# WU-CVGL/Styl3R

Measured on AMD Instinct MI355X. Metric: 256x256 stylized views/sec (fwd+bwd) @ ~65k Gaussians, higher is better.
Workload: dtype f32; 1 GPU; rasterizer fwd+bwd (decoder API + MSE, the loss computed inside the composite kernels): 10 scenes x 4 target views/GPU/step, 256x256, G=65536 Gaussians/scene (1 ctx view x 256x256), sh_degree=0, make_scale_invariant, all views in one batched launch; outputs the decoder discards are not computed (decoder_splatting_cuda.py:37-68 drops radii / opacity / n_touched, MSE sends no depth gradient: the com; parallelism=dp1 (scenes sharded)

## Files before the change

### include/gsr.h

```cpp
#ifndef GSR_H
#define GSR_H

#include <stddef.h>
#include <stdint.h>

#ifdef __cplusplus
extern "C" {
#endif

#define GSR_OK 0
#define GSR_EINVAL (-1)
#define GSR_ENOSPACE (-2)
#define GSR_ELAUNCH (-3)

#define GSR_TILE 16
#define GSR_VIEW_FLOATS 64

typedef struct GsrView {
    float viewmatrix[16];
    float projmatrix[16];
    float projmatrix_raw[16];
    float campos[3];
    float tanfovx, tanfovy;
    float bg[3];
    float scale;
    float pad[7];
} GsrView;

typedef struct GsrDims {
    int32_t B;
    int32_t Vt;
    int32_t G;
    int32_t H, W;
    int32_t M;
    int32_t sh_degree;
    int32_t flags;
    void *profile;
} GsrDims;

#define GSR_FLAG_NTOUCHED 1
#define GSR_FLAG_COV9 2
#define GSR_FLAG_PHASE_BIN 4
#define GSR_FLAG_PHASE_RENDER 8

#define GSR_FLAG_PREZERO_GRADS 16
#define GSR_FLAG_BIN_BALLOT 32
#define GSR_FLAG_SORT_KEYS_SHIFT 8

#define GSR_STATUS_WORDS 8
#define GSR_ST_PAIRS 0
#define GSR_ST_OVERFLOW 1
#define GSR_ST_MAX_TILE 2
#define GSR_ST_PAIRS_HI 3

typedef struct GsrLayout {
    size_t records;
    size_t tile_count;
    size_t tile_offset;
    size_t tile_cursor;
    size_t pairs;
    size_t point_list;
    size_t final_T;
    size_t n_contrib;
    size_t grad_rec;
    size_t status;
    size_t tile_order;
    size_t pairs_alt;
    size_t loss_partial;
    size_t loss_ticket;
    size_t loss_diff;
    size_t total;
} GsrLayout;

#define GSR_ID_MASK 0x0fffffffu
#define GSR_QUAD_SHIFT 28

int gsr_workspace_layout(const GsrDims *dims, int64_t pair_capacity, GsrLayout *out);

int gsr_forward(const GsrDims *dims, const GsrView *views, const float *means, const float *cov6,
                const float *opac, const float *shs, int64_t pair_capacity, void *workspace,
                size_t workspace_bytes, float *image, float *depth, float *opacity, int32_t *radii,
                int32_t *n_touched, int32_t *status, void *stream);

int gsr_backward(const GsrDims *dims, const GsrView *views, const float *means, const float *cov6,
                 const float *shs, int64_t pair_capacity, void *workspace, size_t workspace_bytes,
                 const float *dL_dimage, const float *dL_ddepth, float *dL_dmeans, float *dL_dcov6,
                 float *dL_dopac, float *dL_dshs, float *dL_dmeans2D, float *dL_dtau, void *stream);

typedef struct GsrFused {
    uint32_t *tile_count;
    const float *mse_target;
    float mse_weight;
    float *mse_loss;
    const float *mse_grad_loss;
} GsrFused;
int gsr_forward_fused(const GsrDims *dims, const GsrView *views, const float *means, const float *cov6,
                      const float *opac, const float *shs, int64_t pair_capacity, void *workspace,
                      size_t workspace_bytes, float *image, float *depth, float *opacity, int32_t *radii,
                      int32_t *n_touched, int32_t *status, const GsrFused *fx, void *stream);
int gsr_backward_fused(const GsrDims *dims, const GsrView *views, const float *means, const float *cov6,
                       const float *shs, int64_t pair_capacity, void *workspace, size_t workspace_bytes,
                       const float *dL_dimage, const float *dL_ddepth, float *dL_dmeans, float *dL_dcov6,
                       float *dL_dopac, float *dL_dshs, float *dL_dmeans2D, float *dL_dtau, const GsrFused *fx,
// ... 34 lines not shown
```

### styl3r_amd/_lib.py

```python
from __future__ import annotations

import ctypes as C
import os
import subprocess
from pathlib import Path

_PKG = Path(__file__).resolve().parent
_CSRC = _PKG / "csrc"
_LIBDIR = _PKG / "lib"
LIB_PATH = _LIBDIR / os.environ.get("GSR_LIB_NAME", "libgsr_hip.so")

_SOURCES = ["gsr_forward.hip", "gsr_backward.hip", "gsr_api.hip", "gsr_loss.hip"]
_HEADERS = ["gsr_common.h", "../../include/gsr.h"]

HIPCC_FLAGS = [
    "--offload-arch=gfx950", "-O3", "-std=c++17", "-fPIC", "-shared",
    "-fhip-fp32-correctly-rounded-divide-sqrt", "-fvisibility=hidden",
    "-fno-slp-vectorize",
]


def _hipcc() -> str:
    for cand in (os.environ.get("HIPCC"), "/opt/rocm/bin/hipcc"):
        if cand and os.path.exists(cand):
# ... 18 lines not shown


def build_digest() -> str:
    _, deps, cmd = _build_cmd()
    return sources_digest(deps, cmd)


def built_digest() -> str:
    stamp = LIB_PATH.with_suffix(".stamp")
    return stamp.read_text().strip() if stamp.exists() and LIB_PATH.exists() else ""


def build_library(force: bool = False, verbose: bool = False) -> Path:
    srcs, deps, cmd = _build_cmd()
    _LIBDIR.mkdir(exist_ok=True)
    want = sources_digest(deps, cmd)
    if not force and built_digest() == want:
        return LIB_PATH
    real = [_hipcc(), *cmd[1:-2], "-o", str(LIB_PATH)]
    if verbose:
        print(" ".join(real))
    subprocess.run(real, check=True, cwd=str(_CSRC))
    LIB_PATH.with_suffix(".stamp").write_text(want)
    return LIB_PATH


class GsrDims(C.Structure):
    _fields_ = [("B", C.c_int32), ("Vt", C.c_int32), ("G", C.c_int32), ("H", C.c_int32), ("W", C.c_int32),
                ("M", C.c_int32), ("sh_degree", C.c_int32), ("flags", C.c_int32), ("profile", C.c_void_p)]


class GsrLayout(C.Structure):
    _fields_ = [(n, C.c_size_t) for n in ("records", "tile_count", "tile_offset", "tile_cursor", "pairs", "point_list",
                                          "final_T", "n_contrib", "grad_rec", "status", "tile_order", "pairs_alt", "loss_partial", "loss_ticket", "loss_diff", "total")]


class GsrFused(C.Structure):
    _fields_ = [("tile_count", C.c_void_p), ("mse_target", C.c_void_p), ("mse_weight", C.c_float), ("mse_loss", C.c_void_p),
                ("mse_grad_loss", C.c_void_p)]


GSR_FLAG_NTOUCHED = 1
GSR_FLAG_COV9 = 2
GSR_FLAG_PHASE_BIN = 4
GSR_FLAG_PHASE_RENDER = 8
GSR_FLAG_PREZERO_GRADS = 16
GSR_FLAG_BIN_BALLOT = 32
GSR_ID_MASK = 0x0FFFFFFF
GSR_QUAD_SHIFT = 28
GSR_FLAG_SORT_KEYS_SHIFT = 8
GSR_STATUS_WORDS = 8
GSR_VIEW_FLOATS = 64
GSR_N_STAGES = 7
STAGE_NAMES = ("preprocess", "scan_tiles", "scatter", "tile_sort", "composite_fwd", "composite_bwd", "preprocess_bwd")
EXPORTS = ("gsr_workspace_layout", "gsr_forward", "gsr_backward", "gsr_forward_fused", "gsr_backward_fused", "gsr_version", "gsr_profile_create",
           "gsr_profile_destroy", "gsr_profile_read", "gsr_profile_set_stages", "gsr_last_error", "gsr_build_views", "gsr_mse_scratch_bytes",
           "gsr_mse_forward", "gsr_mse_backward")
ERRORS = {-1: "GSR_EINVAL (bad dimension / null pointer / unsupported degree)",
          -2: "GSR_ENOSPACE (workspace too small)", -3: "GSR_ELAUNCH (kernel launch failed)"}

_lib = None


def load() -> C.CDLL:
    global _lib
    if _lib is not None:
        return _lib
    if not LIB_PATH.exists():
        raise RuntimeError(
            f"{LIB_PATH} is missing: the HIP rasterizer has not been built. "
            "Run `python -c 'import __graft_entry__ as g; g.build()'` (needs hipcc). There is no CPU fallback.")
    import torch
    lib = C.CDLL(str(LIB_PATH))
    vp, i64, sz = C.c_void_p, C.c_int64, C.c_size_t
    lib.gsr_workspace_layout.argtypes = [C.POINTER(GsrDims), i64, C.POINTER(GsrLayout)]
    lib.gsr_workspace_layout.restype = C.c_int
    lib.gsr_forward.argtypes = [C.POINTER(GsrDims), vp, vp, vp, vp, vp, i64, vp, sz, vp, vp, vp, vp, vp, vp, vp]
    lib.gsr_forward.restype = C.c_int
    lib.gsr_backward.argtypes = [C.POINTER(GsrDims), vp, vp, vp, vp, i64, vp, sz, vp, vp, vp, vp, vp, vp, vp, vp, vp]
    lib.gsr_backward.restype = C.c_int
    lib.gsr_forward_fused.argtypes = [C.POINTER(GsrDims), vp, vp, vp, vp, vp, i64, vp, sz, vp, vp, vp, vp, vp, vp, C.POINTER(GsrFused), vp]
    lib.gsr_forward_fused.restype = C.c_int
    lib.gsr_backward_fused.argtypes = [C.POINTER(GsrDims), vp, vp, vp, vp, i64, vp, sz, vp, vp, vp, vp, vp, vp, vp, vp, C.POINTER(GsrFused), vp]
    lib.gsr_backward_fused.restype = C.c_int
# ... 56 lines not shown
```

### styl3r_amd/csrc/gsr_api.hip

```cpp
#include <new>

#include "gsr_common.h"

namespace gsr {
int layout(const GsrDims &d, long long cap, GsrLayout &L);
int forward(const GsrDims &d, const GsrView *views, const float *means, const float *cov6, const float *opac,
            const float *shs, long long cap, void *workspace, size_t workspace_bytes, float *image, float *depth,
            float *opacity, int32_t *radii, int32_t *n_touched, int32_t *status, const GsrFused *fx, hipStream_t stream);
int backward(const GsrDims &d, const GsrView *views, const float *means, const float *cov6, const float *shs,
             long long cap, void *workspace, size_t workspace_bytes, const float *dL_dimage, const float *dL_ddepth,
             float *dL_dmeans, float *dL_dcov6, float *dL_dopac, float *dL_dshs, float *dL_dmeans2D, float *dL_dtau,
             const GsrFused *fx, hipStream_t stream);
}

namespace gsr {
thread_local hipError_t g_last_hip_error = hipSuccess;

#pragma clang fp contract(off)
__device__ inline void inverse4(const float *m, float *inv)
{
    float a[4][8];
#pragma unroll
    for (int r = 0; r < 4; ++r)
#pragma unroll
// ... 195 lines not shown
    if (!p) return;
    const size_t n = (size_t)p->max_calls * GSR_N_STAGES * 2;
    for (size_t i = 0; i < n; ++i)
        if (p->ev[i]) (void)hipEventDestroy(p->ev[i]);
    delete[] p->ev;
    delete p;
}

__attribute__((visibility("default"))) int gsr_profile_read(GsrProfile *p, float *ms_sum, int32_t *count)
{
    if (!p || !ms_sum || !count) return GSR_EINVAL;
    for (int s = 0; s < GSR_N_STAGES; ++s) { ms_sum[s] = 0.f; count[s] = 0; }
    for (int s = 0; s < GSR_N_STAGES; ++s) {
        if (!((p->mask >> s) & 1u)) continue;
        const int n = (s <= GSR_STAGE_COMPOSITE_FWD) ? p->next_fwd : p->next_bwd;
        for (int c = 0; c < n; ++c) {
            float ms = 0.f;
            if (hipEventSynchronize(p->at(c, s, 1)) != hipSuccess) return GSR_ELAUNCH;
            if (hipEventElapsedTime(&ms, p->at(c, s, 0), p->at(c, s, 1)) != hipSuccess) return GSR_ELAUNCH;
            ms_sum[s] += ms; count[s] += 1;
        }
    }
    p->next_fwd = p->next_bwd = 0;
    return GSR_OK;
}

__attribute__((visibility("default"))) int gsr_profile_set_stages(GsrProfile *p, uint32_t stage_mask)
{
    if (!p || p->next_fwd || p->next_bwd) return GSR_EINVAL;
    p->mask = stage_mask & ((1u << GSR_N_STAGES) - 1u);
    return GSR_OK;
}

__attribute__((visibility("default"))) const char *gsr_version(void) { return "gsr-hip gfx950 0.6.0"; }

}
```

### styl3r_amd/csrc/gsr_backward.hip

```cpp
#include <type_traits>

#include "gsr_common.h"

namespace gsr {

enum { GR_RGB = 0, GR_DEPTH = 3, GR_MX = 4, GR_MY = 5, GR_CA = 6, GR_CB = 7, GR_CC = 8, GR_OP = 9 };

template <bool DEPTH>
__global__ void __launch_bounds__(64) k_composite_bwd(GsrDims d, const GsrView *__restrict__ views, Ptrs ws,
                                                     const float *__restrict__ dL_dimage,
                                                     const float *__restrict__ dL_ddepth,
                                                     bool mse, float mse_weight, const float *__restrict__ mse_grad_loss)
{
    if (ws.status[GSR_ST_OVERFLOW]) return;
    __shared__ float4 s_q[64 * 3];

    const int gx = tiles_x(d.W), T = gx * tiles_y(d.H);
    const uint32_t tv = ws.tile_order[blockIdx.y * gridDim.x + blockIdx.x];
    const int tile = (int)(tv % (uint32_t)T), v = (int)(tv / (uint32_t)T);
    const int lane = threadIdx.x;
    const int ox = (tile % gx) * TILE + (lane & 7), oy = (tile / gx) * TILE + (lane >> 3);
    const size_t P = (size_t)d.H * d.W;

    const size_t t = (size_t)v * T + tile;
    const uint32_t start = ws.tile_offset[t], end = ws.tile_offset[t + 1];
    if (start == end) return;
    const uint32_t *__restrict__ plist = ws.point_list + start;
    const SplatRec *__restrict__ recs = ws.records + (size_t)v * d.G;
    float *grad = ws.grad_rec + (size_t)v * d.G * GR_STRIDE;
    const GsrView &vw = views[v];

    const float fx0 = (float)ox, fy0 = (float)oy;
    float Tr[4], g0[4], g1[4], g2[4], gd[4], S[4];
    uint32_t last[4];
    uint32_t mx = 0;
    const float mse_c = mse ? 2.0f * mse_weight / (float)((size_t)d.B * d.Vt * 3 * P) * (mse_grad_loss ? mse_grad_loss[0] : 1.f) : 0.f;
#pragma unroll
    for (int k = 0; k < 4; ++k) {
        const int px = ox + (k & 1) * 8, py = oy + (k >> 1) * 8;
        const bool inside = px < d.W && py < d.H;
        const size_t pix = (size_t)py * d.W + px;
        const float Tf = inside ? ws.final_T[v * P + pix] : 0.f;
        last[k] = inside ? ws.n_contrib[v * P + pix] : 0u;
        g0[k] = (inside && dL_dimage) ? dL_dimage[(v * 3 + 0) * P + pix] : 0.f;
        g1[k] = (inside && dL_dimage) ? dL_dimage[(v * 3 + 1) * P + pix] : 0.f;
        g2[k] = (inside && dL_dimage) ? dL_dimage[(v * 3 + 2) * P + pix] : 0.f;
        if (mse && inside) {
            const float e0 = mse_c * ws.loss_diff[(v * 3 + 0) * P + pix], e1 = mse_c * ws.loss_diff[(v * 3 + 1) * P + pix],
                        e2 = mse_c * ws.loss_diff[(v * 3 + 2) * P + pix];
            if (dL_dimage) { g0[k] += e0; g1[k] += e1; g2[k] += e2; }
            else { g0[k] = e0; g1[k] = e1; g2[k] = e2; }
        }
        gd[k] = (DEPTH && inside) ? dL_ddepth[v * P + pix] : 0.f;
        S[k] = Tf * (vw.bg[0] * g0[k] + vw.bg[1] * g1[k] + vw.bg[2] * g2[k]);
        Tr[k] = Tf;
        mx = max(mx, last[k]);
    }
    const float ddelx_dx = 0.5f * (float)d.W, ddely_dy = 0.5f * (float)d.H;
#pragma unroll
    for (int o = 32; o > 0; o >>= 1) mx = max(mx, (uint32_t)__shfl_xor((int)mx, o, 64));
    const int max_last = __builtin_amdgcn_readfirstlane((int)mx);
    constexpr bool NINE = !DEPTH;
    int slot;
    if (NINE) { const int i9 = reduce9_slot(lane); slot = i9 < 0 ? -1 : (i9 < 3 ? i9 : i9 + 1); }
    else slot = reduce10_slot(lane);

    for (int hi = max_last; hi > 0; hi -= 64) {
        const int cnt = min(64, hi);
        asm volatile("" ::: "memory");
        uint32_t bm = 0;
        if (lane < cnt) {
            const uint32_t word = plist[hi - 1 - lane];
            bm = word >> GSR_QUAD_SHIFT;
            stage_entry_bwd(recs, word & GSR_ID_MASK, bm, s_q + lane * 3);
        }
        unsigned long long todo = __builtin_amdgcn_ballot_w64(bm != 0u);
        asm volatile("s_waitcnt lgkmcnt(0)" ::: "memory");
        for (; todo; todo &= todo - 1ull) {
            const int j = __builtin_ctzll(todo);
            const uint32_t entry = (uint32_t)(hi - 1 - j);
            const float4 a = s_q[j * 3 + 0];
            const float4 b = s_q[j * 3 + 1];
            const float4 c = s_q[j * 3 + 2];
            const uint32_t quad = __builtin_amdgcn_readfirstlane(__float_as_uint(c.w));
            float s[10];
#pragma unroll
            for (int i = 0; i < 10; ++i) asm volatile("" : "=v"(s[i]));
            if (!DEPTH && !NINE) s[GR_DEPTH] = 0.f;
            unsigned long long anym = 0ull;
            auto eval = [&](const bool FIRST, const int k) {
                const float dx = (a.x - fx0) - (float)((k & 1) * 8), dy = (a.y - fy0) - (float)((k >> 1) * 8);
                const float power = -0.5f * (a.z * dx * dx + b.x * dy * dy) - a.w * dx * dy;
                const float Graw = footprint_exp(power);
                const float araw = fminf(0.99f, b.y * Graw);
                const unsigned long long vm = __builtin_amdgcn_ballot_w64(entry < last[k]) & __builtin_amdgcn_ballot_w64(power <= 0.f) &
                                              __builtin_amdgcn_ballot_w64(araw >= (1.f / 255.f));
                anym |= vm;
                const float alpha = sel0_f(vm, araw);
                const float Gv = sel0_f(vm, Graw);
                const float inv = __builtin_amdgcn_rcpf(1.f - alpha);
                Tr[k] *= inv;
// ... 277 lines not shown
        for (int k = 0; k < 3 * NC; ++k) dsh[k] = dsh_acc[k];
        for (int k = 3 * NC; k < ncol; ++k) dsh[k] = 0.f;
    }
}
#pragma clang fp contract(fast)

int layout(const GsrDims &d, long long cap, GsrLayout &L);
Ptrs carve(void *base, const GsrLayout &L);

int backward(const GsrDims &d, const GsrView *views, const float *means, const float *cov6, const float *shs,
             long long cap, void *workspace, size_t workspace_bytes, const float *dL_dimage, const float *dL_ddepth,
             float *dL_dmeans, float *dL_dcov6, float *dL_dopac, float *dL_dshs, float *dL_dmeans2D, float *dL_dtau,
             const GsrFused *fx, hipStream_t stream)
{
    GsrLayout L;
    int rc = layout(d, cap, L);
    if (rc != GSR_OK) return rc;
    const float *mse_target = fx ? fx->mse_target : nullptr;
    if (!views || !means || !cov6 || !shs || !workspace || !dL_dmeans || !dL_dcov6 || !dL_dopac || !dL_dshs) return GSR_EINVAL;
    if (!dL_dimage && !mse_target) return GSR_EINVAL;
    if (workspace_bytes < L.total) return GSR_ENOSPACE;
    Ptrs ws = carve(workspace, L);
    const int V = d.B * d.Vt, T = tiles_x(d.W) * tiles_y(d.H);
    (void)hipGetLastError();
    StageTimer tm(d.profile, false, stream);
    if (!(d.flags & GSR_FLAG_PREZERO_GRADS) &&
        !hip_ok(hipMemsetAsync(ws.grad_rec, 0, (size_t)V * d.G * GR_STRIDE * 4, stream))) return GSR_ELAUNCH;
    if (dL_dtau && !hip_ok(hipMemsetAsync(dL_dtau, 0, (size_t)V * 6 * 4, stream))) return GSR_ELAUNCH;
    tm.begin(GSR_STAGE_COMPOSITE_BWD);
    {
        const float *mg = fx ? fx->mse_grad_loss : nullptr;
        const float mw = fx ? fx->mse_weight : 0.f;
        const bool mse = mse_target != nullptr;
        if (dL_ddepth) hipLaunchKernelGGL(k_composite_bwd<true>, dim3(T, V), dim3(64), 0, stream, d, views, ws, dL_dimage, dL_ddepth, mse, mw, mg);
        else hipLaunchKernelGGL(k_composite_bwd<false>, dim3(T, V), dim3(64), 0, stream, d, views, ws, dL_dimage, dL_ddepth, mse, mw, mg);
    }
    tm.end(GSR_STAGE_COMPOSITE_BWD); tm.begin(GSR_STAGE_PREPROCESS_BWD);
    const dim3 gG((d.G + 255) / 256, d.B);
#define GSR_LAUNCH_K7(DEG) hipLaunchKernelGGL(k_preprocess_bwd<DEG>, gG, dim3(256), 0, stream, d, views, means, cov6, shs, ws, \
                                              dL_dmeans, dL_dcov6, dL_dopac, dL_dshs, dL_dmeans2D, dL_dtau)
    switch (d.M > 0 ? d.sh_degree : -1) {
        case -1: GSR_LAUNCH_K7(-1); break;
        case 0: GSR_LAUNCH_K7(0); break;
        case 1: GSR_LAUNCH_K7(1); break;
        case 2: GSR_LAUNCH_K7(2); break;
        case 3: GSR_LAUNCH_K7(3); break;
        default: GSR_LAUNCH_K7(4); break;
    }
#undef GSR_LAUNCH_K7
    tm.end(GSR_STAGE_PREPROCESS_BWD);
    return launch_status();
}

}
```

### styl3r_amd/csrc/gsr_common.h

```cpp
#pragma once
#include <hip/hip_runtime.h>
#include <stdint.h>

#include "../../include/gsr.h"

namespace gsr {

constexpr int TILE = GSR_TILE;
constexpr int TILE_PIX = TILE * TILE;
constexpr int WAVE = 64;

struct alignas(16) SplatRec {
    float x, y, depth;
    uint32_t rad_flags;
    float A, B, C, opacity;
    float r, g, b;
    uint32_t ext;
};
constexpr int LDS_TILES_MAX = 4096;
static_assert(sizeof(SplatRec) == 48, "SplatRec must be 48 bytes");

struct alignas(16) QueueRec {
    float x, y, A, B;
    float C, opacity, depth; uint32_t id;
    float r, g, b; uint32_t quad;
};
static_assert(sizeof(QueueRec) == 48, "QueueRec must be 48 bytes");

constexpr int GR_STRIDE = 12;

struct Ptrs {
    SplatRec *records;
    uint32_t *tile_count, *tile_offset, *tile_cursor, *tile_order;
    unsigned long long *pairs, *pairs_alt;
    uint32_t *point_list;
    float *loss_partial;
    uint32_t *loss_ticket;
    float *loss_diff;
    float *final_T;
    uint32_t *n_contrib;
    float *grad_rec;
    int32_t *status;
};

}

struct GsrProfile {
    int max_calls;
    int next_fwd, next_bwd;
    uint32_t mask;
    hipEvent_t *ev;
    hipEvent_t &at(int call, int stage, int which) { return ev[((size_t)call * GSR_N_STAGES + stage) * 2 + which]; }
};

namespace gsr {

extern thread_local hipError_t g_last_hip_error;
inline int launch_status()
{
    hipError_t e = hipGetLastError();
    if (e == hipSuccess) return GSR_OK;
    g_last_hip_error = e;
    return GSR_ELAUNCH;
}
inline bool hip_ok(hipError_t e)
{
    if (e == hipSuccess) return true;
    g_last_hip_error = e;
    return false;
}

struct StageTimer {
    GsrProfile *p; int slot; hipStream_t s;
    StageTimer(void *prof, bool fwd, hipStream_t stream, bool resume = false)
        : p(static_cast<GsrProfile *>(prof)), slot(-1), s(stream)
    {
        if (!p) return;
        int &n = fwd ? p->next_fwd : p->next_bwd;
        if (resume) { if (n > 0 && n <= p->max_calls) slot = n - 1; }
        else if (n < p->max_calls) slot = n++;
    }
    void begin(int stage) { if (slot >= 0 && ((p->mask >> stage) & 1u)) (void)hipEventRecord(p->at(slot, stage, 0), s); }
    void end(int stage) { if (slot >= 0 && ((p->mask >> stage) & 1u)) (void)hipEventRecord(p->at(slot, stage, 1), s); }
};

__host__ __device__ inline int tiles_x(int W) { return (W + TILE - 1) / TILE; }
__host__ __device__ inline int tiles_y(int H) { return (H + TILE - 1) / TILE; }

__device__ constexpr float SH_C0 = 0.28209479177387814f;
__device__ constexpr float SH_C1 = 0.4886025119029199f;
__device__ constexpr float SH_C2_0 = 1.0925484305920792f, SH_C2_1 = -1.0925484305920792f, SH_C2_2 = 0.31539156525252005f,
                           SH_C2_3 = -1.0925484305920792f, SH_C2_4 = 0.5462742152960396f;
__device__ constexpr float SH_C3_0 = -0.5900435899266435f, SH_C3_1 = 2.890611442640554f, SH_C3_2 = -0.4570457994644658f,
                           SH_C3_3 = 0.3731763325901154f, SH_C3_4 = -0.4570457994644658f, SH_C3_5 = 1.445305721320277f,
                           SH_C3_6 = -0.5900435899266435f;
__device__ constexpr float SH_C4_0 = 2.5033429417967046f, SH_C4_1 = -1.7701307697799304f, SH_C4_2 = 0.9461746957575601f,
                           SH_C4_3 = -0.6690465435572892f, SH_C4_4 = 0.10578554691520431f, SH_C4_5 = -0.6690465435572892f,
                           SH_C4_6 = 0.47308734787878004f, SH_C4_7 = -1.7701307697799304f, SH_C4_8 = 0.6258357354491761f;

#pragma clang fp contract(off)

__device__ inline void sh_basis(int deg, float x, float y, float z, float *b)
{
    b[0] = SH_C0;
    if (deg < 1) return;
    b[1] = -SH_C1 * y; b[2] = SH_C1 * z; b[3] = -SH_C1 * x;
    if (deg < 2) return;
    float xx = x * x, yy = y * y, zz = z * z, xy = x * y, yz = y * z, xz = x * z;
    b[4] = SH_C2_0 * xy; b[5] = SH_C2_1 * yz; b[6] = SH_C2_2 * (2.0f * zz - xx - yy);
    b[7] = SH_C2_3 * xz; b[8] = SH_C2_4 * (xx - yy);
    if (deg < 3) return;
    b[9] = SH_C3_0 * y * (3.0f * xx - yy);
    b[10] = SH_C3_1 * xy * z;
    b[11] = SH_C3_2 * y * (4.0f * zz - xx - yy);
    b[12] = SH_C3_3 * z * (2.0f * zz - 3.0f * xx - 3.0f * yy);
    b[13] = SH_C3_4 * x * (4.0f * zz - xx - yy);
    b[14] = SH_C3_5 * z * (xx - yy);
    b[15] = SH_C3_6 * x * (xx - 3.0f * yy);
    if (deg < 4) return;
    b[16] = SH_C4_0 * xy * (xx - yy);
// ... 305 lines not shown
```

### styl3r_amd/csrc/gsr_forward.hip

```cpp
#include <cstdlib>
#include <cstring>
#include <type_traits>

#include "gsr_common.h"

namespace gsr {

#pragma clang fp contract(off)
template <int DEG>
__global__ void __launch_bounds__(256) k_preprocess(GsrDims d, const GsrView *__restrict__ views,
                                                    const float *__restrict__ means, const float *__restrict__ cov6,
                                                    const float *__restrict__ opac, const float *__restrict__ shs,
                                                    Ptrs ws, int32_t *__restrict__ radii, int lds_tiles)
{
    extern __shared__ uint32_t s_tiles[];
    const int g = blockIdx.x * blockDim.x + threadIdx.x;
    const int b = blockIdx.y;
    const bool live = g < d.G;
    const size_t sg = (size_t)b * d.G + (live ? g : 0);
    const float m0[3] = {means[3 * sg], means[3 * sg + 1], means[3 * sg + 2]};
    float S0[6];
    load_cov(cov6, sg, (d.flags & GSR_FLAG_COV9) != 0, S0);
    const float op = opac[sg];
    const int gx = tiles_x(d.W), gy = tiles_y(d.H), T = gx * gy;
// ... 78 lines not shown
            const int rw = maxx - minx, area = ok ? rw * (maxy - miny) : 0;
            for (int k = 0; k < area; ++k) atomicAdd(&s_tiles[(miny + k / rw) * gx + minx + k % rw], 1u);
            __syncthreads();
            uint32_t *cnt = ws.tile_count + (size_t)v * T;
            for (int t = threadIdx.x; t < T; t += 256) {
                const uint32_t c = s_tiles[t];
                if (c) { atomicAdd(cnt + t, c); s_tiles[t] = 0u; }
            }
            __syncthreads();
        } else {
            const int rw = maxx - minx, area = ok ? rw * (maxy - miny) : 0;
            int amax = area;
#pragma unroll
            for (int o = 32; o > 0; o >>= 1) amax = max(amax, __shfl_xor(amax, o, 64));
            uint32_t *cnt = ws.tile_count + (size_t)v * T;
            for (int k = 0; k < amax; ++k) {
                const bool has = k < area;
                const int ty = has ? miny + k / rw : 0, tx = has ? minx + k % rw : 0;
                wave_agg_inc<false>(cnt, (uint32_t)(ty * gx + tx), has);
            }
        }
        if (live) {
            float4 *dst = reinterpret_cast<float4 *>(ws.records + vg);
            const float4 *src = reinterpret_cast<const float4 *>(&rec);
            dst[0] = src[0]; dst[1] = src[1]; dst[2] = src[2];
            radii[vg] = rad * (ok ? 1 : 0);
        }
    }
}
#pragma clang fp contract(fast)

constexpr int SCAN_PER_MAX = 16;

__global__ void __launch_bounds__(1024) k_scan_tiles(int n, long long capacity, Ptrs ws, int32_t *__restrict__ status, int rearm, int nticket)
{
    __shared__ unsigned long long s_wave[16];
    __shared__ unsigned long long s_carry;
    __shared__ uint32_t s_max[16];
    __shared__ uint32_t s_bin[256], s_shift;
    __shared__ uint32_t s_cnt[1024 * SCAN_PER_MAX];
    const int tid = threadIdx.x, lane = tid & 63, wid = tid >> 6;
    uint32_t mx = 0;
    const int per = (n + 1023) / 1024;
    const bool fast = per <= SCAN_PER_MAX;
    uint32_t c[SCAN_PER_MAX];
    if (fast) {
        for (int i = tid; i < per * 1024; i += 1024) s_cnt[i] = (i < n) ? ws.tile_count[i] : 0u;
        if (rearm) for (int i = tid; i < n; i += 1024) ws.tile_count[i] = 0u;
        for (int i = tid; i < nticket; i += 1024) ws.loss_ticket[i] = 0u;
        __syncthreads();
        unsigned long long tot = 0;
#pragma unroll
        for (int e = 0; e < SCAN_PER_MAX; ++e) {
            c[e] = (e < per) ? s_cnt[tid * per + e] : 0u;
            mx = max(mx, c[e]);
            tot += c[e];
        }
        unsigned long long x = tot;
#pragma unroll
        for (int o = 1; o < 64; o <<= 1) {
            unsigned long long y = __shfl_up(x, o, 64);
            if (lane >= o) x += y;
        }
        if (lane == 63) s_wave[wid] = x;
        __syncthreads();
        unsigned long long off = x - tot;
        for (int w = 0; w < wid; ++w) off += s_wave[w];
        if (tid == 1023) s_carry = off + tot;
#pragma unroll
        for (int e = 0; e < SCAN_PER_MAX; ++e) {
            const int i = tid * per + e;
            if (e < per && i < n) {
// ... 4 lines not shown
        }
    } else {
        if (tid == 0) s_carry = 0;
        for (int i = tid; i < nticket; i += 1024) ws.loss_ticket[i] = 0u;
        __syncthreads();
        for (int base = 0; base < n; base += 1024) {
            int i = base + tid;
            uint32_t cc = (i < n) ? ws.tile_count[i] : 0u;
            mx = max(mx, cc);
            unsigned long long x = cc;
#pragma unroll
            for (int o = 1; o < 64; o <<= 1) {
                unsigned long long y = __shfl_up(x, o, 64);
                if (lane >= o) x += y;
            }
            if (lane == 63) s_wave[wid] = x;
            __syncthreads();
            unsigned long long wave_off = 0;
            for (int w = 0; w < wid; ++w) wave_off += s_wave[w];
            unsigned long long carry = s_carry;
            unsigned long long excl = carry + wave_off + x - cc;
            if (i < n) {
                ws.tile_offset[i] = (uint32_t)min(excl, (unsigned long long)0xffffffffu);
                ws.tile_cursor[i] = 0u;
            }
            __syncthreads();
            if (tid == 1023) s_carry = carry + wave_off + x;
            __syncthreads();
        }
    }
#pragma unroll
    for (int o = 32; o > 0; o >>= 1) mx = max(mx, (uint32_t)__shfl_xor((int)mx, o, 64));
    if (lane == 0) s_max[wid] = mx;
    if (tid < 256) s_bin[tid] = 0u;
    __syncthreads();
    if (tid == 0) {
        uint32_t m = 0;
        for (int w = 0; w < 16; ++w) m = max(m, s_max[w]);
        unsigned long long R = s_carry;
        ws.tile_offset[n] = (uint32_t)min(R, (unsigned long long)0xffffffffu);
        int ovf = (R > (unsigned long long)capacity || R > 0xffffffffull) ? 1 : 0;
        int32_t st[GSR_STATUS_WORDS] = {(int32_t)(R & 0xffffffffull), ovf, (int32_t)m, (int32_t)(R >> 32), 0, 0, 0, 0};
        for (int k = 0; k < GSR_STATUS_WORDS; ++k) { status[k] = st[k]; ws.status[k] = st[k]; }
        uint32_t sh = 0;
        while ((m >> sh) > 255u) ++sh;
        s_shift = sh;
    }
    __syncthreads();
    const uint32_t sh = s_shift;
    if (fast) {
#pragma unroll
        for (int e = 0; e < SCAN_PER_MAX; ++e)
            if (e < per && tid * per + e < n) atomicAdd(&s_bin[255u - min(c[e] >> sh, 255u)], 1u);
    } else {
        for (int i = tid; i < n; i += 1024) atomicAdd(&s_bin[255u - min(ws.tile_count[i] >> sh, 255u)], 1u);
    }
    __syncthreads();
    if (tid < 64) {
        uint32_t b0 = s_bin[tid * 4], b1 = s_bin[tid * 4 + 1], b2 = s_bin[tid * 4 + 2], b3 = s_bin[tid * 4 + 3];
        uint32_t t4 = b0 + b1 + b2 + b3, x = t4;
#pragma unroll
        for (int o = 1; o < 64; o <<= 1) {
            uint32_t y = (uint32_t)__shfl_up((int)x, o, 64);
            if (lane >= o) x += y;
        }
        uint32_t off = x - t4;
        s_bin[tid * 4] = off; s_bin[tid * 4 + 1] = off + b0; s_bin[tid * 4 + 2] = off + b0 + b1; s_bin[tid * 4 + 3] = off + b0 + b1 + b2;
    }
    __syncthreads();
    if (fast) {
#pragma unroll
        for (int e = 0; e < SCAN_PER_MAX; ++e) {
            const int i = tid * per + e;
            if (e < per && i < n) ws.tile_order[atomicAdd(&s_bin[255u - min(c[e] >> sh, 255u)], 1u)] = (uint32_t)i;
        }
    } else {
        for (int i = tid; i < n; i += 1024) {
            const uint32_t pos = atomicAdd(&s_bin[255u - min(ws.tile_count[i] >> sh, 255u)], 1u);
            ws.tile_order[pos] = (uint32_t)i;
            if (rearm) ws.tile_count[i] = 0u;
        }
    }
}

#pragma clang fp contract(off)
__global__ void __launch_bounds__(256) k_scatter(GsrDims d, Ptrs ws)
{
    if (ws.status[GSR_ST_OVERFLOW]) return;
    const int g = blockIdx.x * blockDim.x + threadIdx.x;
    const int v = blockIdx.y;
    const bool live = g < d.G;
    const size_t vg = (size_t)v * d.G + (live ? g : 0);
    const float4 q0 = reinterpret_cast<const float4 *>(ws.records + vg)[0];
    const int rad = live ? (int)(__float_as_uint(q0.w) & 0xffffffu) : 0;
    const int gx = tiles_x(d.W), gy = tiles_y(d.H), T = gx * gy;
    int minx = 0, miny = 0, maxx = 0, maxy = 0;
    if (rad > 0) tile_rect(q0.x, q0.y, rad, gx, gy, minx, miny, maxx, maxy);
    const unsigned long long key = ((unsigned long long)__float_as_uint(q0.z) << 32) | (unsigned)g;
    const size_t tb = (size_t)v * T;
    const int rw = maxx - minx, area = rw * (maxy - miny);
    int amax = area;
#pragma unroll
    for (int o = 32; o > 0; o >>= 1) amax = max(amax, __shfl_xor(amax, o, 64));
    for (int k = 0; k < amax; ++k) {
        const bool has = k < area;
        const int ty = has ? miny + k / rw : 0, tx = has ? minx + k % rw : 0;
        const uint32_t tl = (uint32_t)(ty * gx + tx);
        const uint32_t slot = wave_agg_inc<true>(ws.tile_cursor + tb, tl, has);
        if (has) ws.pairs[ws.tile_offset[tb + tl] + slot] = key;
    }
}
#pragma clang fp contract(fast)
// ... 280 lines not shown
    const int tile = (int)(tv % (uint32_t)T), v = (int)(tv / (uint32_t)T);
    const int lane = threadIdx.x;
    const int ox = (tile % gx) * TILE + (lane & 7), oy = (tile / gx) * TILE + (lane >> 3);

    if (d.flags & GSR_FLAG_PREZERO_GRADS) {
        const size_t n4 = (size_t)d.B * d.Vt * d.G * (GR_STRIDE / 4);
        const size_t nwg = (size_t)gridDim.x * gridDim.y, wg = (size_t)blockIdx.y * gridDim.x + blockIdx.x;
        const size_t per = (n4 + nwg - 1) / nwg, lo = wg * per, hi = lo + per < n4 ? lo + per : n4;
        float4 *gz = reinterpret_cast<float4 *>(ws.grad_rec);
        for (size_t i = lo + lane; i < hi; i += 64) gz[i] = make_float4(0.f, 0.f, 0.f, 0.f);
    }

    const size_t t = (size_t)v * T + tile;
    const uint32_t start = ws.tile_offset[t];
    const int n = (int)(ws.tile_offset[t + 1] - start);
    uint32_t *__restrict__ plist = ws.point_list + start;
    const SplatRec *__restrict__ recs = ws.records + (size_t)v * d.G;
    const int tile_ox = (tile % gx) * TILE, tile_oy = (tile / gx) * TILE;

    float fx0 = (float)ox, fy0 = (float)oy;
    asm volatile("" : "+v"(fx0), "+v"(fy0));
    float Tr[4], C0[4], C1[4], C2[4], D[4], O[4];
    uint32_t last[4];
    bool inside[4];
    unsigned long long dmask[4];
#pragma unroll
    for (int k = 0; k < 4; ++k) {
        const int px = ox + (k & 1) * 8, py = oy + (k >> 1) * 8;
        inside[k] = px < d.W && py < d.H;
        Tr[k] = 1.f; C0[k] = C1[k] = C2[k] = D[k] = O[k] = 0.f;
        last[k] = 0;
        dmask[k] = __builtin_amdgcn_ballot_w64(!inside[k]);
    }

    for (int base = 0; base < n; base += 64) {
        const int cnt = __builtin_amdgcn_readfirstlane(min(64, n - base));
        __syncthreads();
        uint32_t qm = 0;
        if (lane < cnt) {
            const uint32_t id = plist[base + lane] & GSR_ID_MASK;
            qm = stage_entry_fwd(recs, id, tile_ox, tile_oy, s_q + lane * 3);
            if (qm) plist[base + lane] = id | (qm << GSR_QUAD_SHIFT);
        }
        __syncthreads();

        for (unsigned long long todo = __builtin_amdgcn_ballot_w64(qm != 0u); todo; todo &= todo - 1ull) {
            const int j = __builtin_ctzll(todo);
            const float4 a = s_q[j * 3 + 0];
            const float4 b = s_q[j * 3 + 1];
            const float4 c = s_q[j * 3 + 2];
            const uint32_t quad = __builtin_amdgcn_readfirstlane(__float_as_uint(c.w));
            uint32_t touched_tot = 0;
#pragma unroll
            for (int k = 0; k < 4; ++k) {
                if (!(quad & (1u << k))) continue;
                if (dmask[k] == ~0ull) continue;
                const float dx = (a.x - fx0) - (float)((k & 1) * 8), dy = (a.y - fy0) - (float)((k >> 1) * 8);
                const float power = -0.5f * (a.z * dx * dx + b.x * dy * dy) - a.w * dx * dy;
                const float alpha = fminf(0.99f, b.y * footprint_exp(power));
                const float test_T = Tr[k] * (1.f - alpha);
                const unsigned long long live = __builtin_amdgcn_ballot_w64(!(power > 0.f)) & __builtin_amdgcn_ballot_w64(!(alpha < (1.f / 255.f))) & ~dmask[k];
                const unsigned long long keep = __builtin_amdgcn_ballot_w64(!(test_T < 0.0001f));
                dmask[k] |= live & ~keep;
                const unsigned long long comp = live & keep;
                const float w = sel0_f(comp, alpha * Tr[k]);
                C0[k] += c.x * w; C1[k] += c.y * w; C2[k] += c.z * w;
                D[k] += b.z * w;
                O[k] += w;
                if (NTOUCH) touched_tot += (uint32_t)__popcll(comp & __builtin_amdgcn_ballot_w64(test_T > 0.5f));
                Tr[k] = sel_f(comp, test_T, Tr[k]);
                last[k] = sel_u(comp, (uint32_t)(base + j + 1), last[k]);
            }
            if (NTOUCH) {
                if (touched_tot && lane == 0) atomicAdd(n_touched + (size_t)v * d.G + (__float_as_uint(b.w)), (int)touched_tot);
            }
        }
        if ((dmask[0] & dmask[1] & dmask[2] & dmask[3]) == ~0ull) break;
    }

    const size_t P = (size_t)d.H * d.W;
    const GsrView &vw = views[v];
    float sq = 0.f;
#pragma unroll
    for (int k = 0; k < 4; ++k) {
        if (!inside[k]) continue;
        const size_t pix = (size_t)(oy + (k >> 1) * 8) * d.W + (ox + (k & 1) * 8);
        ws.final_T[v * P + pix] = Tr[k];
        ws.n_contrib[v * P + pix] = last[k];
        const float r0 = C0[k] + Tr[k] * vw.bg[0], r1 = C1[k] + Tr[k] * vw.bg[1], r2 = C2[k] + Tr[k] * vw.bg[2];
        image[(v * 3 + 0) * P + pix] = r0;
        image[(v * 3 + 1) * P + pix] = r1;
        image[(v * 3 + 2) * P + pix] = r2;
        out_depth[v * P + pix] = D[k];
        out_opacity[v * P + pix] = O[k];
        if (mse_target) {
            const float e0 = r0 - mse_target[(v * 3 + 0) * P + pix], e1 = r1 - mse_target[(v * 3 + 1) * P + pix],
                        e2 = r2 - mse_target[(v * 3 + 2) * P + pix];
            sq += (e0 * e0 + e1 * e1) + e2 * e2;
            ws.loss_diff[(v * 3 + 0) * P + pix] = e0; ws.loss_diff[(v * 3 + 1) * P + pix] = e1; ws.loss_diff[(v * 3 + 2) * P + pix] = e2;
        }
    }
    if (!mse_target) return;
    const int V = d.B * d.Vt;
    sq = wave_sum_to_lane63(sq);
    uint32_t arrived = 0;
    if (lane == 63) {
        agent_publish(ws.loss_partial + t, sq);
        asm volatile("s_waitcnt vmcnt(0)" ::: "memory");
        arrived = __hip_atomic_fetch_add(ws.loss_ticket + v, 1u, __ATOMIC_RELAXED, __HIP_MEMORY_SCOPE_AGENT);
    }
    arrived = (uint32_t)__builtin_amdgcn_readlane((int)arrived, 63);
    if (arrived != (uint32_t)T - 1u) return;
    float s1 = 0.f;
    for (int i = lane; i < T; i += 64) s1 += agent_read(ws.loss_partial + (size_t)v * T + i);
    s1 = wave_sum_to_lane63(s1);
    arrived = 0;
    if (lane == 63) {
        agent_publish(ws.loss_partial + (size_t)V * T + v, s1);
        asm volatile("s_waitcnt vmcnt(0)" ::: "memory");
        arrived = __hip_atomic_fetch_add(ws.loss_ticket + V, 1u, __ATOMIC_RELAXED, __HIP_MEMORY_SCOPE_AGENT);
    }
    arrived = (uint32_t)__builtin_amdgcn_readlane((int)arrived, 63);
    if (arrived != (uint32_t)V - 1u) return;
    float s2 = 0.f;
    for (int i = lane; i < V; i += 64) s2 += agent_read(ws.loss_partial + (size_t)V * T + i);
    s2 = wave_sum_to_lane63(s2);
    if (lane == 63) mse_loss[0] = mse_weight * (s2 / (float)((size_t)V * 3 * P));
}

static inline size_t align_up(size_t x, size_t a) { return (x + a - 1) / a * a; }

int layout(const GsrDims &d, long long cap, GsrLayout &L)
{
    if (d.B <= 0 || d.Vt <= 0 || d.G <= 0 || d.H <= 0 || d.W <= 0 || cap <= 0) return GSR_EINVAL;
    if (d.M < 0 || d.sh_degree < 0 || d.sh_degree > 4) return GSR_EINVAL;
    if (d.M > 0 && (d.sh_degree + 1) * (d.sh_degree + 1) > d.M) return GSR_EINVAL;
    if (d.M == 0 && d.sh_degree != 0) return GSR_EINVAL;
    if (cap > 0xffffffffll) return GSR_EINVAL;
    if ((long long)d.G * (long long)sizeof(SplatRec) > 0xffffffffll) return GSR_EINVAL;
    static_assert((0xffffffffull / sizeof(SplatRec)) < GSR_ID_MASK, "ids must leave the quadrant-mask bits of a point_list word free");
    const size_t V = (size_t)d.B * d.Vt, T = (size_t)tiles_x(d.W) * tiles_y(d.H), P = (size_t)d.H * d.W;
    size_t off = 0;
    auto take = [&](size_t bytes) { size_t o = off; off = align_up(off + bytes, 256); return o; };
    L.records = take(V * d.G * sizeof(SplatRec));
    L.tile_count = take(V * T * 4);
    L.tile_offset = take((V * T + 1) * 4);
    L.tile_cursor = take(V * T * 4);
    L.pairs = take((size_t)cap * 8);
    L.point_list = take((size_t)cap * 4);
    L.final_T = take(V * P * 4);
    L.n_contrib = take(V * P * 4);
    L.grad_rec = take(V * d.G * 12 * 4);
    L.status = take(GSR_STATUS_WORDS * 4);
    L.tile_order = take(V * T * 4);
    L.pairs_alt = take((size_t)cap * 8);
    L.loss_partial = take((V * T + V) * 4);
    L.loss_ticket = take((V + 1) * 4);
    L.loss_diff = take(V * 3 * P * 4);
    L.total = off;
    return GSR_OK;
}

Ptrs carve(void *base, const GsrLayout &L)
{
    char *p = static_cast<char *>(base);
    Ptrs w;
    w.records = reinterpret_cast<SplatRec *>(p + L.records);
    w.tile_count = reinterpret_cast<uint32_t *>(p + L.tile_count);
    w.tile_offset = reinterpret_cast<uint32_t *>(p + L.tile_offset);
    w.tile_cursor = reinterpret_cast<uint32_t *>(p + L.tile_cursor);
    w.pairs = reinterpret_cast<unsigned long long *>(p + L.pairs);
    w.point_list = reinterpret_cast<uint32_t *>(p + L.point_list);
    w.final_T = reinterpret_cast<float *>(p + L.final_T);
    w.n_contrib = reinterpret_cast<uint32_t *>(p + L.n_contrib);
    w.grad_rec = reinterpret_cast<float *>(p + L.grad_rec);
    w.status = reinterpret_cast<int32_t *>(p + L.status);
    w.tile_order = reinterpret_cast<uint32_t *>(p + L.tile_order);
    w.pairs_alt = reinterpret_cast<unsigned long long *>(p + L.pairs_alt);
    w.loss_partial = reinterpret_cast<float *>(p + L.loss_partial);
    w.loss_ticket = reinterpret_cast<uint32_t *>(p + L.loss_ticket);
    w.loss_diff = reinterpret_cast<float *>(p + L.loss_diff);
    return w;
}

int forward(const GsrDims &d, const GsrView *views, const float *means, const float *cov6, const float *opac,
            const float *shs, long long cap, void *workspace, size_t workspace_bytes, float *image, float *depth,
            float *opacity, int32_t *radii, int32_t *n_touched, int32_t *status, const GsrFused *fx, hipStream_t stream)
{
    GsrLayout L;
    int rc = layout(d, cap, L);
    if (rc != GSR_OK) return rc;
    if (!views || !means || !cov6 || !opac || !shs || !workspace || !image || !depth || !opacity || !radii || !status)
        return GSR_EINVAL;
    const bool ntouch = (d.flags & GSR_FLAG_NTOUCHED) != 0;
    if (ntouch && !n_touched) return GSR_EINVAL;
    if (workspace_bytes < L.total) return GSR_ENOSPACE;
    const float *mse_target = fx ? fx->mse_target : nullptr;
    if (mse_target && !fx->mse_loss) return GSR_EINVAL;
    Ptrs ws = carve(workspace, L);
    const bool persistent_counters = fx && fx->tile_count;
    if (persistent_counters) ws.tile_count = fx->tile_count;
    const int V = d.B * d.Vt, gx = tiles_x(d.W), gy = tiles_y(d.H), T = gx * gy;
    (void)hipGetLastError();
    const bool bin = (d.flags & GSR_FLAG_PHASE_BIN) != 0, render = (d.flags & GSR_FLAG_PHASE_RENDER) != 0;
    if (bin && render) return GSR_EINVAL;
    StageTimer tm(d.profile, true, stream, render);
    const dim3 gG((d.G + 255) / 256, d.B), gV((d.G + 255) / 256, V);
    const int lds_tiles = (T <= LDS_TILES_MAX && !(d.flags & GSR_FLAG_BIN_BALLOT)) ? T : 0;
    if (render) goto render_phase;

    if (!persistent_counters && !hip_ok(hipMemsetAsync(ws.tile_count, 0, (size_t)V * T * 4, stream))) return GSR_ELAUNCH;
    if (ntouch && !hip_ok(hipMemsetAsync(n_touched, 0, (size_t)V * d.G * 4, stream))) return GSR_ELAUNCH;

    tm.begin(GSR_STAGE_PREPROCESS);
#define GSR_LAUNCH_K1(DEG) hipLaunchKernelGGL(k_preprocess<DEG>, gG, dim3(256), lds_tiles * 4, stream, d, views, means, cov6, opac, shs, ws, radii, lds_tiles)
    switch (d.M > 0 ? d.sh_degree : -1) {
        case -1: GSR_LAUNCH_K1(-1); break;
        case 0: GSR_LAUNCH_K1(0); break;
        case 1: GSR_LAUNCH_K1(1); break;
        case 2: GSR_LAUNCH_K1(2); break;
        case 3: GSR_LAUNCH_K1(3); break;
        default: GSR_LAUNCH_K1(4); break;
    }
#undef GSR_LAUNCH_K1
    tm.end(GSR_STAGE_PREPROCESS); tm.begin(GSR_STAGE_SCAN);
    hipLaunchKernelGGL(k_scan_tiles, dim3(1), dim3(1024), 0, stream, V * T, cap, ws, status, persistent_counters ? 1 : 0, mse_target ? V + 1 : 0);
    tm.end(GSR_STAGE_SCAN);
    if (bin) return launch_status();
render_phase:
    tm.begin(GSR_STAGE_SCATTER);
    if (lds_tiles) hipLaunchKernelGGL(k_scatter_lds, gV, dim3(256), lds_tiles * 8, stream, d, ws);
    else hipLaunchKernelGGL(k_scatter, gV, dim3(256), 0, stream, d, ws);
    tm.end(GSR_STAGE_SCATTER); tm.begin(GSR_STAGE_SORT);
    {
        const int sel = (d.flags >> GSR_FLAG_SORT_KEYS_SHIFT) & 3;
        const uint32_t lds_keys = sel == 1 ? 1024u : (sel == 2 ? 2048u : SORT_LDS_KEYS);
        hipLaunchKernelGGL(k_tile_sort, dim3(T, V), dim3(256), lds_keys * 8, stream, d, ws, lds_keys);
    }
    tm.end(GSR_STAGE_SORT); tm.begin(GSR_STAGE_COMPOSITE_FWD);
    {
        const float mse_weight = fx ? fx->mse_weight : 0.f;
        float *mse_loss = fx ? fx->mse_loss : nullptr;
        if (ntouch) hipLaunchKernelGGL(k_composite_fwd<true>, dim3(T, V), dim3(64), 0, stream, d, views, ws, image, depth, opacity, n_touched, mse_target, mse_weight, mse_loss);
        else hipLaunchKernelGGL(k_composite_fwd<false>, dim3(T, V), dim3(64), 0, stream, d, views, ws, image, depth, opacity, n_touched, mse_target, mse_weight, mse_loss);
    }
    tm.end(GSR_STAGE_COMPOSITE_FWD);
    return launch_status();
}

}
```

Baseline: 29470 views/s.

## Split backward composite into checkpointed per-tile segments for load balance

The forward composite now checkpoints per-pixel transmittance and accumulated colour/depth every seg Gaussians, and stores final colour. The scan kernel builds a unit_order list of (tile, segment) work units sorted by remaining length. The backward composite launches one block per unit and replays only its segment from the checkpoint, so long tiles are split across many blocks instead of serialising in one. This costs extra checkpoint and final-colour writes in the forward pass, more workspace, and more scan-kernel work.

```diff
diff --git a/include/gsr.h b/include/gsr.h
--- a/include/gsr.h
+++ b/include/gsr.h
@@ -46,12 +46,14 @@
 #define GSR_FLAG_PREZERO_GRADS 16
 #define GSR_FLAG_BIN_BALLOT 32
 #define GSR_FLAG_SORT_KEYS_SHIFT 8
+#define GSR_FLAG_SEG_SHIFT 10
 
 #define GSR_STATUS_WORDS 8
 #define GSR_ST_PAIRS 0
 #define GSR_ST_OVERFLOW 1
 #define GSR_ST_MAX_TILE 2
 #define GSR_ST_PAIRS_HI 3
+#define GSR_ST_UNITS 4
 
 typedef struct GsrLayout {
     size_t records;
@@ -69,6 +71,9 @@
     size_t loss_partial;
     size_t loss_ticket;
     size_t loss_diff;
+    size_t final_C;
+    size_t ckpt;
+    size_t unit_order;
     size_t total;
 } GsrLayout;
 
diff --git a/styl3r_amd/_lib.py b/styl3r_amd/_lib.py
--- a/styl3r_amd/_lib.py
+++ b/styl3r_amd/_lib.py
@@ -74,7 +74,8 @@
 
 class GsrLayout(C.Structure):
     _fields_ = [(n, C.c_size_t) for n in ("records", "tile_count", "tile_offset", "tile_cursor", "pairs", "point_list",
-                                          "final_T", "n_contrib", "grad_rec", "status", "tile_order", "pairs_alt", "loss_partial", "loss_ticket", "loss_diff", "total")]
+                                          "final_T", "n_contrib", "grad_rec", "status", "tile_order", "pairs_alt", "loss_partial", "loss_ticket", "loss_diff", "final_C", "ckpt", "unit_order",
+                                          "total")]
 
 
 class GsrFused(C.Structure):
@@ -91,7 +92,9 @@
 GSR_ID_MASK = 0x0FFFFFFF
 GSR_QUAD_SHIFT = 28
 GSR_FLAG_SORT_KEYS_SHIFT = 8
+GSR_FLAG_SEG_SHIFT = 10
 GSR_STATUS_WORDS = 8
+GSR_ST_UNITS = 4
 GSR_VIEW_FLOATS = 64
 GSR_N_STAGES = 7
 STAGE_NAMES = ("preprocess", "scan_tiles", "scatter", "tile_sort", "composite_fwd", "composite_bwd", "preprocess_bwd")
diff --git a/styl3r_amd/csrc/gsr_api.hip b/styl3r_amd/csrc/gsr_api.hip
--- a/styl3r_amd/csrc/gsr_api.hip
+++ b/styl3r_amd/csrc/gsr_api.hip
@@ -251,6 +251,6 @@
     return GSR_OK;
 }
 
-__attribute__((visibility("default"))) const char *gsr_version(void) { return "gsr-hip gfx950 0.6.0"; }
-
-}
+__attribute__((visibility("default"))) const char *gsr_version(void) { return "gsr-hip gfx950 0.7.0"; }
+
+}
diff --git a/styl3r_amd/csrc/gsr_backward.hip b/styl3r_amd/csrc/gsr_backward.hip
--- a/styl3r_amd/csrc/gsr_backward.hip
+++ b/styl3r_amd/csrc/gsr_backward.hip
@@ -13,10 +13,12 @@
                                                      bool mse, float mse_weight, const float *__restrict__ mse_grad_loss)
 {
     if (ws.status[GSR_ST_OVERFLOW]) return;
+    if (blockIdx.x >= (uint32_t)ws.status[GSR_ST_UNITS]) return;
     __shared__ float4 s_q[64 * 3];
 
     const int gx = tiles_x(d.W), T = gx * tiles_y(d.H);
-    const uint32_t tv = ws.tile_order[blockIdx.y * gridDim.x + blockIdx.x];
+    const uint2 unit = ws.unit_order[blockIdx.x];
+    const uint32_t tv = unit.x;
     const int tile = (int)(tv % (uint32_t)T), v = (int)(tv / (uint32_t)T);
     const int lane = threadIdx.x;
     const int ox = (tile % gx) * TILE + (lane & 7), oy = (tile / gx) * TILE + (lane >> 3);
@@ -60,13 +62,32 @@
 #pragma unroll
     for (int o = 32; o > 0; o >>= 1) mx = max(mx, (uint32_t)__shfl_xor((int)mx, o, 64));
     const int max_last = __builtin_amdgcn_readfirstlane((int)mx);
+    const uint32_t seg = seg_len(d);
+    const int lo = (int)(unit.y * seg);
+    if (lo >= max_last) return;
+    int top = max_last;
+    if ((uint32_t)lo + seg < (uint32_t)max_last) {
+        top = lo + (int)seg;
+        const float *slot = ws.ckpt + (size_t)(start / seg + unit.y) * CKPT_SLOT_FLOATS;
+#pragma unroll
+        for (int k = 0; k < 4; ++k) {
+            const int px = ox + (k & 1) * 8, py = oy + (k >> 1) * 8;
+            if (px < d.W && py < d.H) {
+                const float4 cb = reinterpret_cast<const float4 *>(slot)[k * 64 + lane];
+                const float4 cf = ws.final_C[v * P + (size_t)py * d.W + px];
+                Tr[k] = cb.x;
+                S[k] += g0[k] * (cf.x - cb.y) + g1[k] * (cf.y - cb.z) + g2[k] * (cf.z - cb.w);
+                if (DEPTH) S[k] += gd[k] * (cf.w - slot[4 * TILE_PIX + k * 64 + lane]);
+            }
+        }
+    }
     constexpr bool NINE = !DEPTH;
     int slot;
     if (NINE) { const int i9 = reduce9_slot(lane); slot = i9 < 0 ? -1 : (i9 < 3 ? i9 : i9 + 1); }
     else slot = reduce10_slot(lane);
 
-    for (int hi = max_last; hi > 0; hi -= 64) {
-        const int cnt = min(64, hi);
+    for (int hi = top; hi > lo; hi -= 64) {
+        const int cnt = min(64, hi - lo);
         asm volatile("" ::: "memory");
         uint32_t bm = 0;
         if (lane < cnt) {
@@ -410,8 +431,9 @@
         const float *mg = fx ? fx->mse_grad_loss : nullptr;
         const float mw = fx ? fx->mse_weight : 0.f;
         const bool mse = mse_target != nullptr;
-        if (dL_ddepth) hipLaunchKernelGGL(k_composite_bwd<true>, dim3(T, V), dim3(64), 0, stream, d, views, ws, dL_dimage, dL_ddepth, mse, mw, mg);
-        else hipLaunchKernelGGL(k_composite_bwd<false>, dim3(T, V), dim3(64), 0, stream, d, views, ws, dL_dimage, dL_ddepth, mse, mw, mg);
+        const dim3 grid((uint32_t)unit_capacity((size_t)V * T, cap, seg_len(d)));
+        if (dL_ddepth) hipLaunchKernelGGL(k_composite_bwd<true>, grid, dim3(64), 0, stream, d, views, ws, dL_dimage, dL_ddepth, mse, mw, mg);
+        else hipLaunchKernelGGL(k_composite_bwd<false>, grid, dim3(64), 0, stream, d, views, ws, dL_dimage, dL_ddepth, mse, mw, mg);
     }
     tm.end(GSR_STAGE_COMPOSITE_BWD); tm.begin(GSR_STAGE_PREPROCESS_BWD);
     const dim3 gG((d.G + 255) / 256, d.B);
diff --git a/styl3r_amd/csrc/gsr_common.h b/styl3r_amd/csrc/gsr_common.h
--- a/styl3r_amd/csrc/gsr_common.h
+++ b/styl3r_amd/csrc/gsr_common.h
@@ -41,6 +41,9 @@
     uint32_t *n_contrib;
     float *grad_rec;
     int32_t *status;
+    float4 *final_C;
+    float *ckpt;
+    uint2 *unit_order;
 };
 
 }
@@ -86,6 +89,26 @@
 
 __host__ __device__ inline int tiles_x(int W) { return (W + TILE - 1) / TILE; }
 __host__ __device__ inline int tiles_y(int H) { return (H + TILE - 1) / TILE; }
+
+constexpr uint32_t SEG_ONE = 1u << 30;
+constexpr int CKPT_SLOT_FLOATS = 5 * TILE_PIX;
+__host__ __device__ inline uint32_t seg_len(const GsrDims &d)
+{
+    switch ((d.flags >> GSR_FLAG_SEG_SHIFT) & 7) {
+        case 1: return 64u;
+        case 2: return 128u;
+        case 3: return 192u;
+        case 4: return 256u;
+        case 5: return 384u;
+        case 7: return SEG_ONE;
+        default: {
+            const long long vt = (long long)d.B * d.Vt * tiles_x(d.W) * tiles_y(d.H);
+            return vt >= 4096 ? 256u : (vt >= 1024 ? 128u : 64u);
+        }
+    }
+}
+__host__ __device__ inline size_t unit_capacity(size_t VT, long long cap, uint32_t L) { return VT + (size_t)cap / L; }
+__host__ __device__ inline size_t ckpt_slots(long long cap, uint32_t L) { return (size_t)cap / L; }
 
 __device__ constexpr float SH_C0 = 0.28209479177387814f;
 __device__ constexpr float SH_C1 = 0.4886025119029199f;
diff --git a/styl3r_amd/csrc/gsr_forward.hip b/styl3r_amd/csrc/gsr_forward.hip
--- a/styl3r_amd/csrc/gsr_forward.hip
+++ b/styl3r_amd/csrc/gsr_forward.hip
@@ -134,12 +134,14 @@
 
 constexpr int SCAN_PER_MAX = 16;
 
-__global__ void __launch_bounds__(1024) k_scan_tiles(int n, long long capacity, Ptrs ws, int32_t *__restrict__ status, int rearm, int nticket)
+__global__ void __launch_bounds__(1024) k_scan_tiles(int n, long long capacity, Ptrs ws, int32_t *__restrict__ status, int rearm, int nticket,
+                                                     uint32_t seg, uint32_t umax)
 {
     __shared__ unsigned long long s_wave[16];
     __shared__ unsigned long long s_carry;
     __shared__ uint32_t s_max[16];
     __shared__ uint32_t s_bin[256], s_shift;
+    __shared__ uint32_t s_ubin[256], s_ushift, s_ovf, s_units, s_full, s_fcur, s_fw[16];
     __shared__ uint32_t s_cnt[1024 * SCAN_PER_MAX];
     const int tid = threadIdx.x, lane = tid & 63, wid = tid >> 6;
     uint32_t mx = 0;
@@ -210,7 +212,7 @@
 #pragma unroll
     for (int o = 32; o > 0; o >>= 1) mx = max(mx, (uint32_t)__shfl_xor((int)mx, o, 64));
     if (lane == 0) s_max[wid] = mx;
-    if (tid < 256) s_bin[tid] = 0u;
+    if (tid < 256) { s_bin[tid] = 0u; s_ubin[tid] = 0u; }
     __syncthreads();
     if (tid == 0) {
         uint32_t m = 0;
@@ -223,19 +225,67 @@
         uint32_t sh = 0;
         while ((m >> sh) > 255u) ++sh;
         s_shift = sh;
-    }
-    __syncthreads();
-    const uint32_t sh = s_shift;
+        const uint32_t um = min(m, seg);
+        sh = 0;
+        while ((um >> sh) > 255u) ++sh;
+        s_ushift = sh;
+        s_ovf = (uint32_t)ovf;
+        s_full = 0u; s_fcur = 0u;
+    }
+    __syncthreads();
+    const uint32_t sh = s_shift, ush = s_ushift;
+    const bool units = s_ovf == 0u;
+    auto ucls = [&](uint32_t len) { return 255u - min(len >> ush, 255u); };
+    auto nfull = [&](uint32_t cnt) { return cnt ? (cnt - 1u) / seg : 0u; };
+    uint32_t fbase = 0;
+    if (units && fast) {
+        uint32_t fs = 0;
+#pragma unroll
+        for (int e = 0; e < SCAN_PER_MAX; ++e) if (e < per) fs += nfull(c[e]);
+        uint32_t x = fs;
+#pragma unroll
+        for (int o = 1; o < 64; o <<= 1) {
+            const uint32_t y = (uint32_t)__shfl_up((int)x, o, 64);
+            if (lane >= o) x += y;
+        }
+        if (lane == 63) s_fw[wid] = x;
+        __syncthreads();
+        fbase = x - fs;
+        for (int w = 0; w < wid; ++w) fbase += s_fw[w];
+        if (tid == 1023) s_full = fbase + fs;
+    }
+    auto ucount = [&](uint32_t cnt) {
+        if (!units || cnt == 0u) return;
+        if (!fast && cnt > seg) atomicAdd(&s_full, nfull(cnt));
+        atomicAdd(&s_ubin[ucls(cnt - nfull(cnt) * seg)], 1u);
+    };
+    auto uplace = [&](uint32_t i, uint32_t cnt) {
+        if (!units || cnt == 0u) return;
+        const uint32_t nf = nfull(cnt);
+        if (nf) {
+            const uint32_t p = fast ? fbase : atomicAdd(&s_fcur, nf);
+            fbase += nf;
+            for (uint32_t s = 0; s < nf; ++s)
+                if (p + s < umax) ws.unit_order[p + s] = make_uint2(i, s);
+        }
+        const uint32_t p = s_full + atomicAdd(&s_ubin[ucls(cnt - nf * seg)], 1u);
+        if (p < umax) ws.unit_order[p] = make_uint2(i, nf);
+    };
     if (fast) {
 #pragma unroll
         for (int e = 0; e < SCAN_PER_MAX; ++e)
-            if (e < per && tid * per + e < n) atomicAdd(&s_bin[255u - min(c[e] >> sh, 255u)], 1u);
+            if (e < per && tid * per + e < n) { atomicAdd(&s_bin[255u - min(c[e] >> sh, 255u)], 1u); ucount(c[e]); }
     } else {
-        for (int i = tid; i < n; i += 1024) atomicAdd(&s_bin[255u - min(ws.tile_count[i] >> sh, 255u)], 1u);
-    }
-    __syncthreads();
-    if (tid < 64) {
-        uint32_t b0 = s_bin[tid * 4], b1 = s_bin[tid * 4 + 1], b2 = s_bin[tid * 4 + 2], b3 = s_bin[tid * 4 + 3];
+        for (int i = tid; i < n; i += 1024) {
+            const uint32_t cnt = ws.tile_count[i];
+            atomicAdd(&s_bin[255u - min(cnt >> sh, 255u)], 1u);
+            ucount(cnt);
+        }
+    }
+    __syncthreads();
+    if (tid < 128) {
+        uint32_t *bins = tid < 64 ? s_bin : s_ubin;
+        uint32_t b0 = bins[lane * 4], b1 = bins[lane * 4 + 1], b2 = bins[lane * 4 + 2], b3 = bins[lane * 4 + 3];
         uint32_t t4 = b0 + b1 + b2 + b3, x = t4;
 #pragma unroll
         for (int o = 1; o < 64; o <<= 1) {
@@ -243,19 +293,26 @@
             if (lane >= o) x += y;
         }
         uint32_t off = x - t4;
-        s_bin[tid * 4] = off; s_bin[tid * 4 + 1] = off + b0; s_bin[tid * 4 + 2] = off + b0 + b1; s_bin[tid * 4 + 3] = off + b0 + b1 + b2;
-    }
-    __syncthreads();
+        bins[lane * 4] = off; bins[lane * 4 + 1] = off + b0; bins[lane * 4 + 2] = off + b0 + b1; bins[lane * 4 + 3] = off + b0 + b1 + b2;
+        if (tid == 127) s_units = x;
+    }
+    __syncthreads();
+    if (tid == 0) { status[GSR_ST_UNITS] = (int32_t)(s_full + s_units); ws.status[GSR_ST_UNITS] = (int32_t)(s_full + s_units); }
     if (fast) {
 #pragma unroll
         for (int e = 0; e < SCAN_PER_MAX; ++e) {
             const int i = tid * per + e;
-            if (e < per && i < n) ws.tile_order[atomicAdd(&s_bin[255u - min(c[e] >> sh, 255u)], 1u)] = (uint32_t)i;
+            if (e < per && i < n) {
+                ws.tile_order[atomicAdd(&s_bin[255u - min(c[e] >> sh, 255u)], 1u)] = (uint32_t)i;
+                uplace((uint32_t)i, c[e]);
+            }
         }
     } else {
         for (int i = tid; i < n; i += 1024) {
-            const uint32_t pos = atomicAdd(&s_bin[255u - min(ws.tile_count[i] >> sh, 255u)], 1u);
+            const uint32_t cnt = ws.tile_count[i];
+            const uint32_t pos = atomicAdd(&s_bin[255u - min(cnt >> sh, 255u)], 1u);
             ws.tile_order[pos] = (uint32_t)i;
+            uplace((uint32_t)i, cnt);
             if (rearm) ws.tile_count[i] = 0u;
         }
     }
@@ -602,6 +659,8 @@
         last[k] = 0;
         dmask[k] = __builtin_amdgcn_ballot_w64(!inside[k]);
     }
+    const uint32_t seg = seg_len(d);
+    uint32_t ck_next = seg, ck_slot = start / seg;
 
     for (int base = 0; base < n; base += 64) {
         const int cnt = __builtin_amdgcn_readfirstlane(min(64, n - base));
@@ -645,6 +704,15 @@
                 if (touched_tot && lane == 0) atomicAdd(n_touched + (size_t)v * d.G + (__float_as_uint(b.w)), (int)touched_tot);
             }
         }
+        if ((uint32_t)(base + 64) == ck_next && ck_next < (uint32_t)n) {
+            float *slot = ws.ckpt + (size_t)ck_slot * CKPT_SLOT_FLOATS;
+#pragma unroll
+            for (int k = 0; k < 4; ++k) {
+                reinterpret_cast<float4 *>(slot)[k * 64 + lane] = make_float4(Tr[k], C0[k], C1[k], C2[k]);
+                slot[4 * TILE_PIX + k * 64 + lane] = D[k];
+            }
+            ck_next += seg; ++ck_slot;
+        }
         if ((dmask[0] & dmask[1] & dmask[2] & dmask[3]) == ~0ull) break;
     }
 
@@ -663,6 +731,7 @@
         image[(v * 3 + 2) * P + pix] = r2;
         out_depth[v * P + pix] = D[k];
         out_opacity[v * P + pix] = O[k];
+        if ((uint32_t)n > seg) ws.final_C[v * P + pix] = make_float4(C0[k], C1[k], C2[k], D[k]);
         if (mse_target) {
             const float e0 = r0 - mse_target[(v * 3 + 0) * P + pix], e1 = r1 - mse_target[(v * 3 + 1) * P + pix],
                         e2 = r2 - mse_target[(v * 3 + 2) * P + pix];
@@ -727,6 +796,10 @@
     L.loss_partial = take((V * T + V) * 4);
     L.loss_ticket = take((V + 1) * 4);
     L.loss_diff = take(V * 3 * P * 4);
+    const uint32_t seg = seg_len(d);
+    L.final_C = take(seg == SEG_ONE ? 0 : V * P * 16);
+    L.ckpt = take(ckpt_slots(cap, seg) * CKPT_SLOT_FLOATS * 4);
+    L.unit_order = take(unit_capacity(V * T, cap, seg) * 8);
     L.total = off;
     return GSR_OK;
 }
@@ -750,6 +823,9 @@
     w.loss_partial = reinterpret_cast<float *>(p + L.loss_partial);
     w.loss_ticket = reinterpret_cast<uint32_t *>(p + L.loss_ticket);
     w.loss_diff = reinterpret_cast<float *>(p + L.loss_diff);
+    w.final_C = reinterpret_cast<float4 *>(p + L.final_C);
+    w.ckpt = reinterpret_cast<float *>(p + L.ckpt);
+    w.unit_order = reinterpret_cast<uint2 *>(p + L.unit_order);
     return w;
 }
 
@@ -794,7 +870,11 @@
     }
 #undef GSR_LAUNCH_K1
     tm.end(GSR_STAGE_PREPROCESS); tm.begin(GSR_STAGE_SCAN);
-    hipLaunchKernelGGL(k_scan_tiles, dim3(1), dim3(1024), 0, stream, V * T, cap, ws, status, persistent_counters ? 1 : 0, mse_target ? V + 1 : 0);
+    {
+        const uint32_t seg = seg_len(d);
+        hipLaunchKernelGGL(k_scan_tiles, dim3(1), dim3(1024), 0, stream, V * T, cap, ws, status, persistent_counters ? 1 : 0, mse_target ? V + 1 : 0,
+                           seg, (uint32_t)unit_capacity((size_t)V * T, cap, seg));
+    }
     tm.end(GSR_STAGE_SCAN);
     if (bin) return launch_status();
 render_phase:
```

After: 29970 views/s, median of 6. 1.02x the previous value.
